# JettHuang/jet-pbrt

Measured on AMD Instinct MI355X. Metric: Msamples/sec (whole node) + per-pixel L2 vs CPU ref, cornell_box 1024spp, higher is better.
Workload: dtype f32

## Files before the change

### jet-pbrt_amd/csrc/jp_kernels.hip

```cpp
#include "jp_common.h"
#include "jp_tex.h"
#include "jp_env.h"
#include "jp_mis.h"
#include "jp_xbsdf.h"

#include <cstdio>
#include <cstring>
#include <string>
#include <vector>
#include <algorithm>
#include <cmath>
#include <mutex>
#include <thread>
#include "jp_devmem.h"
#include "jp_lbvh.h"
#include "jp_ploc.h"

__global__ void __launch_bounds__(JP_BLOCK) k_raygen(SceneView sc, Queues q, RenderConst rc, DevCounters* cnt)
{
	const unsigned int total = (unsigned int)rc.npix * rc.sbatch;
	const unsigned int nchunks = (total + JP_BLOCK - 1) / JP_BLOCK;
	const unsigned int G = gridDim.x, b = blockIdx.x;
	if (b == 0 && threadIdx.x == 0) { cnt->n_queue[0] = total; cnt->n_queue[1] = 0; cnt->n_shadow = 0; }
	unsigned int filled = 0;
// ... 61 lines not shown
		prims = nodes + 5 * sc.n_nodes;
		for (int i = threadIdx.x; i < 4 * sc.n_nodes; i += JP_BLOCK) nodes[5 * (i >> 2) + (i & 3)] = sc.nodes[i];
		for (int i = threadIdx.x; i < 4 * sc.n_prims; i += JP_BLOCK) prims[5 * (i >> 2) + (i & 3)] = sc.prims[i];
		__syncthreads();
	}
	template <bool kAnyHit> __device__ __forceinline__ int trace(const SceneView&, V3 o, V3 d, float tmin, float& tmax) const
	{ return traverse<kAnyHit, 5>(nodes, prims, o, d, tmin, tmax, stack); }
};
template <typename F> struct SceneAccess<2, F>
{
	float4* prims;
	__device__ __forceinline__ SceneAccess(const SceneView& sc, int)
	{
		prims = s_dyn;
		for (int i = threadIdx.x; i < 4 * sc.n_prims; i += JP_BLOCK) prims[5 * (i >> 2) + (i & 3)] = sc.prims[i];
		__syncthreads();
	}
	template <bool kAnyHit> __device__ __forceinline__ int trace(const SceneView& sc, V3 o, V3 d, float tmin, float& tmax) const
	{ return traverse_flat<kAnyHit, 5, F>(sc.flat, sc.n_flat, sc.n_prims, prims, o, d, tmin, tmax); }
	__device__ __forceinline__ int trace_unbounded(const SceneView& sc, V3 o, V3 d, float tmin, float& tmax) const
	{ return traverse_flat<false, 5, F, true>(sc.flat, sc.n_flat, sc.n_prims, prims, o, d, tmin, tmax); }
};

template <> struct SceneAccess<3>
{
	const float4* prims; unsigned int* stack;
	__device__ __forceinline__ SceneAccess(const SceneView& sc, int) : prims(sc.prims), stack((unsigned int*)s_dyn + threadIdx.x) {}
	template <bool kAnyHit> __device__ __forceinline__ int trace(const SceneView& sc, V3 o, V3 d, float tmin, float& tmax) const
	{ return traverse_wide<kAnyHit>(sc.wide, prims, o, d, tmin, tmax, stack); }
};

template <> struct SceneAccess<4>
{
	WalkStack stack;
	__device__ __forceinline__ SceneAccess(const SceneView&, int depth) { stack.lds = (int*)s_dyn + threadIdx.x; stack.spill = nullptr; stack.cap = depth - 1; stack.stride = 0; }
	template <bool kAnyHit> __device__ __forceinline__ int trace(const SceneView& sc, V3 o, V3 d, float tmin, float& tmax) const
	{ return walk_ray<4, kAnyHit>(sc, o, d, tmin, tmax, stack); }
};

template <> struct SceneAccess<6>
{
	WalkStack stack;
	__device__ __forceinline__ SceneAccess(const SceneView&, int depth) { stack.lds = (int*)s_dyn + threadIdx.x; stack.spill = nullptr; stack.cap = depth - 1; stack.stride = 0; }
	template <bool kAnyHit> __device__ __forceinline__ int trace(const SceneView& sc, V3 o, V3 d, float tmin, float& tmax) const
	{ return walk_ray<6, kAnyHit>(sc, o, d, tmin, tmax, stack); }
};

template <> struct SceneAccess<5>
{
	const float4 *nodes, *prims; int* stack;
	__device__ __forceinline__ SceneAccess(const SceneView& sc, int) : nodes(sc.nodes), prims(sc.prims), stack((int*)s_dyn + threadIdx.x) {}
	template <bool kAnyHit> __device__ __forceinline__ int trace(const SceneView&, V3 o, V3 d, float tmin, float& tmax) const
	{ return traverse_ref<kAnyHit>(nodes, prims, o, d, tmin, tmax, stack); }
};

template <int kMode, typename F = FeatAll>
__global__ void __launch_bounds__(JP_BLOCK) k_extend(SceneView sc, Queues q, int cur, int depth, DevCounters* cnt)
{
	SceneAccess<kMode, F> acc(sc, depth);
	const unsigned int b = blockIdx.x, n = q.blk_q[cur][b], rbase = b * q.R;
	if (b == 0 && threadIdx.x == 0) { cnt->closest += cnt->n_queue[cur]; cnt->n_queue[cur ^ 1] = 0; cnt->n_shadow = 0; }
	unsigned int h = 0;
	float4 ro = make_float4(0, 0, 0, 0), rd = make_float4(0, 0, 1, 0);
	if (threadIdx.x < n) { ro = q.ray_o[cur][rbase + threadIdx.x]; rd = q.ray_d[cur][rbase + threadIdx.x]; }
	for (unsigned int j = threadIdx.x; j < n; j += JP_BLOCK)
	{
		const unsigned int i = rbase + j;
		const float4 co = ro, cd = rd;
		if (j + JP_BLOCK < n) { ro = q.ray_o[cur][i + JP_BLOCK]; rd = q.ray_d[cur][i + JP_BLOCK]; }
		float tmax = JP_INF;
		int hit;
		if constexpr (kMode == 2) hit = acc.trace_unbounded(sc, xyz(co), xyz(cd), 0.001f, tmax);
		else hit = acc.template trace<false>(sc, xyz(co), xyz(cd), 0.001f, tmax);
		q.hit[i] = make_float2(tmax, __int_as_float(hit));
		h += hit >= 0 ? 1u : 0u;
	}
	for (int off = 32; off > 0; off >>= 1) h += __shfl_down(h, off);
	if ((threadIdx.x & 63) == 0 && h) atomicAdd(&cnt->closest_hit, (unsigned long long)h);
}

#ifndef JP_SHADE_TILE
#define JP_SHADE_TILE 8192
#endif
template <bool kTab, bool kPrims, bool kStage, bool kSort, bool kTex, bool kPick, bool kEnv, bool kMis, typename F = FeatAll>
__device__ __forceinline__ void shade_body(SceneView sc, Queues q, RenderConst rc, int cur, DevCounters* cnt, const TexView& tv, const PickView& pv, const EnvView& ev, const MisView& mv)
{
	static_assert(kPick || !kMis, "k_shade: the light strategy's pdf needs the light table");
	static_assert(kTab || !kPrims, "k_shade: primitive records in LDS only together with the tables");
	static_assert(kPick || !kEnv, "k_shade: the map light is an entry of the light table");
	constexpr int kWaves = JP_BLOCK / 64, kMaxSeg = (JP_SHADE_TILE / JP_BLOCK) * kWaves;
	static_assert(JP_SHADE_TILE % JP_BLOCK == 0 && JP_SHADE_TILE <= 65536, "k_shade: tile positions are 16-bit");
	__shared__ unsigned short s_idx[kSort ? JP_SHADE_TILE : 1];
	__shared__ unsigned char s_key[kSort ? JP_SHADE_TILE : 1];
	__shared__ unsigned int s_cnt[kSort ? JP_SHADE_CLASSES * kMaxSeg : 1];
	__shared__ unsigned int s_wsum[kWaves];
	__shared__ unsigned int s_ctr[3];
	const unsigned int lane = threadIdx.x & 63u;
	const int n_tab_l = kPick ? 0 : 2 * sc.n_lights;
	const int n_tab = n_tab_l + 4 * sc.n_mats + (sc.n_mats + 3) / 4, n_tab_all = n_tab + (kPrims ? 8 * sc.n_prims : 0);
	float4* s_lights = s_dyn;
	float4* s_mats = s_lights + n_tab_l;
	int* s_mtype = (int*)(s_mats + 4 * sc.n_mats);
	float4* s_prims = s_dyn + n_tab;
	int4* s_meta = (int4*)(s_prims + 4 * sc.n_prims);
	const float4* s_frames = s_prims + 5 * sc.n_prims;
	float4* s_stage = s_dyn + n_tab_all + threadIdx.x;
	const unsigned int b = blockIdx.x, n = q.blk_q[cur][b];
	const int nxt = cur ^ 1;
#ifdef JP_SHADE_TIMING
	unsigned long long t_acc[10] = { 0, 0, 0, 0, 0, 0, 0, 0, 0, 0 }, t_last = __builtin_amdgcn_s_memtime();
#endif
	if (kTab)
	{
		for (int i = threadIdx.x; i < n_tab_all; i += 2 * JP_BLOCK)
		{
			const bool two = i + JP_BLOCK < n_tab_all;
			const float4 a = sc.shade_tab[i], c2 = two ? sc.shade_tab[i + JP_BLOCK] : a;
			s_dyn[i] = a; if (two) s_dyn[i + JP_BLOCK] = c2;
		}
	}
	if (n == 0) { if (threadIdx.x == 0) { q.blk_q[nxt][b] = 0; q.blk_sh[b] = 0; } return; }
	if (threadIdx.x == 0) { s_ctr[0] = 0; s_ctr[1] = 0; s_ctr[2] = 0; }
	__syncthreads();
	const float4* lights = (kTab && !kPick) ? (const float4*)s_lights : sc.lights;
	const float4* mats = kTab ? (const float4*)s_mats : sc.mats;
	const int* mat_type = kTab ? (const int*)s_mtype : sc.mat_type;
	const float4* prims = kPrims ? (const float4*)s_prims : sc.prims;
	const int4* meta_t = kPrims ? (const int4*)s_meta : sc.meta;
	const unsigned int rbase = b * q.R;
	const unsigned int t0 = 0, count = n;
	JP_TS(0);
	if (kSort)
	{
		constexpr unsigned int seg = kMaxSeg, nctr = JP_SHADE_CLASSES * kMaxSeg;
		const unsigned int tid = threadIdx.x;
		const unsigned int plane = tid & 63u, wave = tid >> 6, npass = (count + JP_BLOCK - 1) / JP_BLOCK;
		const unsigned long long ltm = (1ull << plane) - 1ull;
		#pragma unroll 1
		for (unsigned int r0 = 0; r0 < npass; r0 += 8)
		{
			int pi[8];
			#pragma unroll
			for (int u = 0; u < 8; u++)
			{
				const unsigned int j = (r0 + u) * JP_BLOCK + tid;
				pi[u] = j < count ? __float_as_int(q.hit[rbase + t0 + j].y) : -2;
			}
			#pragma unroll
			for (int u = 0; u < 8; u++)
			{
				const unsigned int r = r0 + u;
				if (r >= npass) break;
				unsigned int key = JP_SHADE_CLASSES;
				if (pi[u] != -2)
				{
					int m = -1; if (pi[u] >= 0) m = meta_t[pi[u]].y;
					key = m >= 0 ? 1u + (unsigned int)mat_type[m] : 0u;
				}
				s_key[r * JP_BLOCK + tid] = (unsigned char)key;
				unsigned int mine = 0;
				#pragma unroll
				for (int c = 0; c < JP_SHADE_CLASSES; c++)
				{
					unsigned int nc = 0;
					if ((rc.class_mask >> c) & 1) nc = (unsigned int)__popcll(__ballot(key == (unsigned int)c));
					if (plane == (unsigned int)c) mine = nc;
				}
				if (plane < JP_SHADE_CLASSES) s_cnt[plane * seg + r * kWaves + wave] = mine;
			}
		}
		__syncthreads();
		{
			static_assert(JP_SHADE_CLASSES * kMaxSeg <= 3 * JP_BLOCK, "k_shade: three counters per thread");
			unsigned int v[3], t = 0;
			#pragma unroll
			for (int i = 0; i < 3; i++)
			{
				const unsigned int at = 3 * tid + i;
				v[i] = (at < nctr && (at % seg) / kWaves < npass) ? s_cnt[at] : 0u; t += v[i];
			}
			unsigned int incl = t;
			#pragma unroll
			for (int off = 1; off < 64; off <<= 1) { const unsigned int o = __shfl_up(incl, off); if (plane >= (unsigned int)off) incl += o; }
			if (plane == 63) s_wsum[wave] = incl;
			__syncthreads();
			unsigned int base = incl - t;
			#pragma unroll
			for (int w = 0; w < kWaves; w++) if ((unsigned int)w < wave) base += s_wsum[w];
			#pragma unroll
			for (int i = 0; i < 3; i++) { const unsigned int at = 3 * tid + i; if (at < nctr) s_cnt[at] = base; base += v[i]; }
		}
		__syncthreads();
		#pragma unroll 1
		for (unsigned int r = 0; r < npass; r++)
		{
			const unsigned int key = s_key[r * JP_BLOCK + tid];
			unsigned int pre = 0;
			#pragma unroll
			for (int c = 0; c < JP_SHADE_CLASSES; c++)
			{
				if (!((rc.class_mask >> c) & 1)) continue;
				const unsigned long long m = __ballot(key == (unsigned int)c);
				if (key == (unsigned int)c) pre = (unsigned int)__popcll(m & ltm);
			}
			if (key < JP_SHADE_CLASSES) s_idx[s_cnt[key * seg + r * kWaves + wave] + pre] = (unsigned short)(r * JP_BLOCK + tid);
		}
		__syncthreads();
	}
	float4 ro_n = make_float4(0, 0, 0, 0), rd_n = ro_n, rb_n = ro_n; float2 h_n = make_float2(0, 0); unsigned int s_n = 0; float2 m_n = make_float2(0, 0);
	JP_TS(1);
	const unsigned int nch = (count + 63u) >> 6;
	unsigned int tk = wave_take(&s_ctr[0], 1u);
	unsigned int c0 = (nch - 1u - tk) << 6;
	if (tk < nch && c0 + lane < count) { const unsigned int pos = c0 + lane, i0 = rbase + t0 + (kSort ? (unsigned int)s_idx[pos] : pos); ro_n = q.ray_o[cur][i0]; rd_n = q.ray_d[cur][i0]; rb_n = q.beta[cur][i0]; h_n = q.hit[i0]; if (kTex) s_n = tv.side[i0]; if (kMis) m_n = mv.side[cur][i0]; }
	while (tk < nch)
	{
		const bool valid = c0 + lane < count;
#ifdef JP_SHADE_TIMING
		JP_TS(2);
		asm volatile("s_waitcnt vmcnt(0)" ::: "memory");
		JP_TS(3);
#endif
#ifdef JP_SHADE_NO_PREFETCH
		if (valid) { const unsigned int pos = c0 + lane, i0 = rbase + t0 + (kSort ? (unsigned int)s_idx[pos] : pos); ro_n = q.ray_o[cur][i0]; rd_n = q.ray_d[cur][i0]; rb_n = q.beta[cur][i0]; h_n = q.hit[i0]; if (kTex) s_n = tv.side[i0]; if (kMis) m_n = mv.side[cur][i0]; }
		const float4 ro = ro_n, rd = rd_n, rb = rb_n; const float2 h = h_n; const unsigned int sw = s_n; const float2 ms = m_n;
		tk = wave_take(&s_ctr[0], 1u); c0 = (nch - 1u - tk) << 6;
#else
		const float4 ro = ro_n, rd = rd_n, rb = rb_n; const float2 h = h_n; const unsigned int sw = s_n; const float2 ms = m_n;
		tk = wave_take(&s_ctr[0], 1u); c0 = (nch - 1u - tk) << 6;
		if (tk < nch && c0 + lane < count)
		{
			const unsigned int pos = c0 + lane;
			const unsigned int i1 = rbase + t0 + (kSort ? (unsigned int)s_idx[pos] : pos);
			ro_n = q.ray_o[cur][i1]; rd_n = q.ray_d[cur][i1]; rb_n = q.beta[cur][i1]; h_n = q.hit[i1]; if (kTex) s_n = tv.side[i1]; if (kMis) m_n = mv.side[cur][i1];
		}
#endif
		bool shaded = false, wantNee = false, alive = false;
		V3 o = mk(0, 0, 0), d = mk(0, 0, 1), beta = mk(0, 0, 0), p = mk(0, 0, 0), N = mk(0, 0, 1);
		int slot = 0, bounce = 0; bool spec = false; unsigned int dim = 0; uint32_t key = 0;
		Closure c; c.kind = CL_LAMBERT; Frame fr; fr.s = fr.t = fr.n = mk(0, 0, 1);
		float2 nm = make_float2(0.f, 0.f);
		if (valid)
		{
			o = xyz(ro); d = xyz(rd); beta = xyz(rb);
			slot = __float_as_int(ro.w); key = (uint32_t)__float_as_int(rb.w);
			const int flags = __float_as_int(rd.w);
			bounce = FLAG_BOUNCE(flags); spec = FLAG_SPEC(flags); dim = FLAG_DIM(flags);
			const int pi = __float_as_int(h.y);
			const bool found = pi >= 0;
			int mat = -1, hitprim = 0; bool nflip = false, tabframe = kPrims;
			V3 Le = splat(0);
			float wLe = 1.f;
			if (found)
			{
				const float4 g3 = prims[4 * pi + 3];
				const int4 meta = meta_t[pi];
				const int type = __float_as_int(g3.w);
				p = o + h.x * d;
				if (type == JP_SHAPE_TRIANGLE) N = xyz(g3);
				else if (!F::curved || type == JP_SHAPE_RECTANGLE) { nflip = !(dot(xyz(g3), d) <= 0); N = nflip ? -xyz(g3) : xyz(g3); }
				else if (type == JP_SHAPE_DISK) N = xyz(prims[4 * pi + 1]);
				else { const float4 g0 = prims[4 * pi]; N = normalize(p - xyz(g0)); tabframe = false; }
				hitprim = pi;
				mat = meta.y;
				if (meta.z >= 0 && (bounce == 0 || spec))
				{
					const V3 wo = -d;
					if (dot(N, wo) > 0.f) Le = xyz(lights[2 * meta.z]);
				}
				else if (kMis && meta.z >= 0)
				{
					const V3 wo = -d;
					if (dot(N, wo) > 0.f)
					{
						Le = xyz(lights[2 * meta.z]);
						if (!isblack(Le))
						{
							bool unweighed;
							const float a = light_pdf(sc, prims, lights, pv, ev, kEnv, meta.z, o - ms.y * d, d, ms.y + h.x, N, unweighed);
							wLe = unweighed ? 0.f : (a > 0.f ? mis_weight(ms.x, a) : 1.f);
						}
					}
				}
			}
			else if (F::other_lights && (bounce == 0 || spec))
			{
				if (kEnv)
				{
					const float4 t = ev.texel[env_lookup(ev, d)];
					float4 L = q.lacc[slot];
					V3 a = mk(L.x, L.y, L.z) + cmul(beta, xyz(t));
					q.lacc[slot] = make_float4(a.x, a.y, a.z, 0.f);
				}
				else if (kPick)
				{
					for (int e = 0; e < pv.n_env; e++)
					{
						float4 L = q.lacc[slot];
						V3 a = mk(L.x, L.y, L.z) + cmul(beta, xyz(pv.env[e]));
						q.lacc[slot] = make_float4(a.x, a.y, a.z, 0.f);
					}
				}
				else for (int li = 0; li < sc.n_lights; li++)
				{
					const float4 l0 = lights[2 * li];
					if (__float_as_int(l0.w) == JP_LIGHT_ENVIRONMENT && !isblack(xyz(l0)))
					{
						float4 L = q.lacc[slot];
						V3 a = mk(L.x, L.y, L.z) + cmul(beta, xyz(l0));
						q.lacc[slot] = make_float4(a.x, a.y, a.z, 0.f);
					}
				}
			}
			else if (kMis)
			{
// ... 104 lines not shown
							s_stage[(2 * k) * JP_BLOCK] = make_float4(sdir.x, sdir.y, sdir.z, dist - 0.001f);
							s_stage[(2 * k + 1) * JP_BLOCK] = make_float4(contrib.x, contrib.y, contrib.z, 0.f);
						}
						else
						{
							q.sh_d[(size_t)k * q.cap + qs] = make_float4(sdir.x, sdir.y, sdir.z, dist - 0.001f);
							q.sh_c[(size_t)k * q.cap + qs] = make_float4(contrib.x, contrib.y, contrib.z, 0.f);
						}
						k++;
					}
				}
				if (!kStage) q.sh_o[qs] = make_float4(p.x, p.y, p.z, __int_as_float(slot | (k << rc.slot_bits)));
			}
		}
		JP_TS(5);
#ifdef JP_DBG_SKIP_SAMPLE
		if (false)
#else
		if (shaded)
#endif
		{
			const float ux = rngf(rc, key, dim), uy = rngf(rc, key, dim + 1); dim += 2;
			BsdfSample bs = sample_local<F>(c, wo, ux, uy);
			bs.wi = to_world(fr, bs.wi);
			if (!(isblack(bs.f) || bs.pdf == 0.f))
			{
				nspec = (bs.flags & BS_SPECULAR) != 0;
				if (bounce >= 3)
				{
					const float qq = smax(0.05f, 1 - maxcomp(bs.f));
					const float ur = rngf(rc, key, dim++);
					if (!(ur < qq))
					{
						nbeta = cmul(beta, bs.f * absdot(bs.wi, N) / (bs.pdf * (1 - qq)));
						alive = true;
					}
				}
				else
				{
					nbeta = cmul(beta, bs.f * absdot(bs.wi, N) / bs.pdf);
					alive = true;
				}
				nd = bs.wi; nbounce = bounce + 1;
				if (kMis) nm = make_float2(bs.pdf, 0.f);
			}
		}
		JP_TS(6);
		unsigned int j = 0;
		const unsigned long long lt = (1ull << lane) - 1ull;
		const unsigned long long ma = __ballot(alive);
		if (kStage)
		{
			const unsigned long long ms = __ballot(k > 0);
			if (ma | ms)
			{
				const unsigned int base = wave_take(&s_ctr[1], (unsigned int)__popcll(ma) | ((unsigned int)__popcll(ms) << 16));
				j = rbase + (base & 0xffffu) + (unsigned int)__popcll(ma & lt);
				qs = rbase + (base >> 16) + (unsigned int)__popcll(ms & lt);
			}
			if (k > 0)
			{
				q.sh_o[qs] = make_float4(p.x, p.y, p.z, __int_as_float(slot | (k << rc.slot_bits)));
				for (int kk = 0; kk < k; kk++)
				{
					q.sh_d[(size_t)kk * q.cap + qs] = s_stage[(2 * kk) * JP_BLOCK];
					q.sh_c[(size_t)kk * q.cap + qs] = s_stage[(2 * kk + 1) * JP_BLOCK];
				}
			}
		}
		else if (ma) j = rbase + wave_take(&s_ctr[1], (unsigned int)__popcll(ma)) + (unsigned int)__popcll(ma & lt);
		if (alive)
		{
			q.ray_o[nxt][j] = make_float4(p.x, p.y, p.z, __int_as_float(slot));
			q.ray_d[nxt][j] = make_float4(nd.x, nd.y, nd.z, __int_as_float(MK_FLAGS(nbounce, nspec, dim)));
			q.beta[nxt][j] = make_float4(nbeta.x, nbeta.y, nbeta.z, __int_as_float((int)key));
			if (kMis) mv.side[nxt][j] = nm;
		}
		JP_TS(7);
#ifdef JP_SHADE_TIMING
		asm volatile("s_waitcnt vmcnt(0)" ::: "memory");
		JP_TS(9);
#endif
	}
	JP_TS(2);
	__syncthreads();
	JP_TS(8);
#ifdef JP_SHADE_TIMING
	if (lane == 0) for (int i = 0; i < 10; i++) atomicAdd(&g_shade_t[i], t_acc[i]);
	if (lane == 0) atomicAdd(&g_shade_t[15], 1ull);
#endif
	if (threadIdx.x == 0)
	{
		const unsigned int run_q = kStage ? (s_ctr[1] & 0xffffu) : s_ctr[1], run_sh = kStage ? (s_ctr[1] >> 16) : s_ctr[2];
		q.blk_q[nxt][b] = run_q; q.blk_sh[b] = run_sh;
		if (run_q) atomicAdd(&cnt->n_queue[nxt], run_q);
		if (run_sh) atomicAdd(&cnt->n_shadow, run_sh);
	}
}
template <bool kTab, bool kPrims, bool kStage, bool kSort, typename F = FeatAll>
__global__ void __launch_bounds__(JP_BLOCK) k_shade(SceneView sc, Queues q, RenderConst rc, int cur, DevCounters* cnt)
{
	const TexView tv = {}; const PickView pv = {}; const EnvView ev = {}; const MisView mv = {};
	shade_body<kTab, kPrims, kStage, kSort, false, false, false, false, F>(sc, q, rc, cur, cnt, tv, pv, ev, mv);
}

template <int kMode, typename F = FeatAll>
__global__ void __launch_bounds__(JP_BLOCK, 4) k_shadow(SceneView sc, Queues q, RenderConst rc, int depth, DevCounters* cnt)
{
#ifdef JP_TRAV_TIMING
	unsigned long long t_acc[10] = { 0, 0, 0, 0, 0, 0, 0, 0, 0, 0 }, t_last = __builtin_amdgcn_s_memtime();
#endif
	SceneAccess<kMode, F> acc(sc, depth);
	const unsigned int b = blockIdx.x, E = q.blk_sh[b], rbase = b * q.R;
	JP_TT(0);
	unsigned int rays = 0, occ = 0;
	float4 so_n = make_float4(0, 0, 0, 0), sd_n = make_float4(0, 0, 1, 0);
	if (threadIdx.x < E) { so_n = q.sh_o[rbase + threadIdx.x]; sd_n = q.sh_d[rbase + threadIdx.x]; }
	for (unsigned int j = threadIdx.x; j < E; j += JP_BLOCK)
	{
		const unsigned int e = rbase + j;
#ifdef JP_TRAV_TIMING
		JP_TT(1);
		asm volatile("s_waitcnt vmcnt(0)" ::: "memory");
		JP_TT(2);
#endif
		const float4 so = so_n; float4 sd = sd_n;
		if (j + JP_BLOCK < E) { so_n = q.sh_o[e + JP_BLOCK]; sd_n = q.sh_d[e + JP_BLOCK]; }
		const int packed = __float_as_int(so.w);
		const int slot = packed & ((1 << rc.slot_bits) - 1), n = (int)((unsigned int)packed >> rc.slot_bits);
		if (n == 0) continue;
		bool any = false;
		const float4 L = q.lacc[slot];
		V3 a = mk(L.x, L.y, L.z);
		for (int k = 0; k < n; k++)
		{
			const float4 c4 = q.sh_c[(size_t)k * q.cap + e];
			float tmax = sd.w;
			const V3 dir = xyz(sd);
			if (k + 1 < n) sd = q.sh_d[(size_t)(k + 1) * q.cap + e];
			JP_TT(3);
#ifdef JP_TRAV_TIMING
			int hit;
			if constexpr (kMode == 2)
			{
				unsigned int m;
				if constexpr (F::curved) m = flat_boxes<false>(sc.flat, sc.n_flat, xyz(so), dir, 0.001f, tmax);
				else m = flat_boxes_lean<false>(sc.flat, sc.n_flat, xyz(so), dir, 0.001f, tmax);
				JP_TT(4);
				hit = flat_prims<true, false, 5, F>(m, acc.prims, xyz(so), dir, 0.001f, tmax);
				JP_TT(5);
			}
			else hit = acc.template trace<true>(sc, xyz(so), dir, 0.001f, tmax);
#else
			const int hit = acc.template trace<true>(sc, xyz(so), dir, 0.001f, tmax);
#endif
			rays++;
			if (hit >= 0) occ++;
			else { a = a + xyz(c4); any = true; }
			JP_TT(6);
		}
		if (any) q.lacc[slot] = make_float4(a.x, a.y, a.z, 0.f);
		JP_TT(7);
	}
#ifdef JP_TRAV_TIMING
	JP_TT(1);
	if ((threadIdx.x & 63) == 0) { for (int i = 0; i < 8; i++) atomicAdd(&g_shade_t[i], t_acc[i]); atomicAdd(&g_shade_t[15], 1ull); }
#endif
	for (int off = 32; off > 0; off >>= 1) { rays += __shfl_down(rays, off); occ += __shfl_down(occ, off); }
	if ((threadIdx.x & 63) == 0) { if (rays) atomicAdd(&cnt->shadow, (unsigned long long)rays); if (occ) atomicAdd(&cnt->shadow_occ, (unsigned long long)occ); }
}

template <int kMode, bool kAnyHit, bool kVote>
__device__ __forceinline__ void persist_turn(Walker<kMode>& w, const SceneView& sc, const WalkStack& stack, bool pool)
{
	const int nh = __popcll(__ballot(!w.done && w.heavy())), nl = __popcll(__ballot(!w.done && !w.heavy()));
	const bool heavyTurn = kVote ? nh > nl : w.heavy();
	if (kVote) { JP_TURN(heavyTurn ? 3 : 0, 1); JP_TURN(heavyTurn ? 4 : 1, heavyTurn ? nh : nl); JP_TURN(heavyTurn ? 5 : 2, nh + nl); if (!pool) { JP_TURN(8, 1); JP_TURN(9, nh + nl); JP_TURN(10, heavyTurn ? nh : nl); } }
	if (!w.done && (w.heavy() == heavyTurn)) w.template step<kAnyHit>(sc, stack);
}
__device__ __forceinline__ unsigned int lane_rank(unsigned long long m) { return __builtin_amdgcn_mbcnt_hi((unsigned int)(m >> 32), __builtin_amdgcn_mbcnt_lo((unsigned int)m, 0u)); }

#ifndef JP_CERT_WAVES
#define JP_CERT_WAVES 8
#endif
template <int kMode, int kRefill, bool kVote>
__global__ void __launch_bounds__(JP_BLOCK, (kMode == 6 ? JP_CERT_WAVES : 8)) k_extend_persist(SceneView sc, Queues q, int cur_q, int stack_cap, int* spill, DevCounters* cnt)
// ... 477 lines not shown
```

### jet-pbrt_amd/csrc/jp_render.h

```cpp
#pragma once
namespace
{
enum { CLS_EXTEND = 0, CLS_SHADE = 1, CLS_SHADOW = 2, CLS_OTHER = 3, CLS_PATH = 4 };

void free_queues(JpContext* c) { c->qb = QueueBufs(); c->cap = 0; c->planes_alloc = 0; c->blk_alloc = 0; }

int ensure_queues(JpContext* c, unsigned int cap, int planes, unsigned int nblocks)
{
	if (c->cap >= cap && c->planes_alloc >= planes && c->blk_alloc >= nblocks) return JP_OK;
	cap = std::max(cap, c->cap); planes = std::max(planes, c->planes_alloc); nblocks = std::max(nblocks, c->blk_alloc);
	free_queues(c);
	auto alloc = [](DevBuf& b, auto*& p, size_t bytes) { return reserve(b, p, bytes) == hipSuccess; };
	Queues& q = c->q; QueueBufs& qb = c->qb; bool ok = true;
	for (int b = 0; b < 2 && ok; b++) ok = alloc(qb.ray_o[b], q.ray_o[b], (size_t)cap * 16) && alloc(qb.ray_d[b], q.ray_d[b], (size_t)cap * 16) && alloc(qb.beta[b], q.beta[b], (size_t)cap * 16)
	                                       && alloc(qb.blk_q[b], q.blk_q[b], (size_t)nblocks * 4);
	ok = ok && alloc(qb.hit, q.hit, (size_t)cap * 8) && alloc(qb.lacc, q.lacc, (size_t)cap * 16) && alloc(qb.sh_o, q.sh_o, (size_t)cap * 16)
	     && alloc(qb.sh_d, q.sh_d, (size_t)cap * 16 * planes) && alloc(qb.sh_c, q.sh_c, (size_t)cap * 16 * planes) && alloc(qb.blk_sh, q.blk_sh, (size_t)nblocks * 4);
	if (!ok) { free_queues(c); return fail(JP_ERR_DEVICE, "jp_render: out of device memory for the path queues"); }
	c->cap = cap; c->planes_alloc = planes; c->blk_alloc = nblocks;
	return JP_OK;
}

int ensure_gamma(JpContext* c)
{
// ... 28 lines not shown
{
	if (rp->width <= 0 || rp->height <= 0 || rp->spp <= 0 || rp->max_depth < 0 || rp->max_depth > 200) return fail(JP_ERR_INVALID_ARGUMENT, "jp_render: bad width/height/spp/max_depth");
	if (rp->integrator < JP_INTEGRATOR_PATH || rp->integrator > JP_INTEGRATOR_DEBUG_NORMAL) return fail(JP_ERR_INVALID_ARGUMENT, "jp_render: unknown integrator");
	if (rp->integrator == JP_INTEGRATOR_WHITTED && rp->max_depth > JP_WHITTED_MAX_DEPTH) return fail(JP_ERR_UNSUPPORTED, "jp_render: the Whitted integrator supports max_depth <= 16");
	if (rp->sampler_mode != JP_SAMPLER_COUNTER && rp->sampler_mode != JP_SAMPLER_DEBUG) return fail(JP_ERR_UNSUPPORTED, "jp_render: the device path implements the counter sampler only (the sequential mt19937_64 stream is not reproducible in parallel)");
	s.band = rp->band_rows > 0 ? rp->band_rows : 20;
	s.count = rp->shard_count > 1 ? rp->shard_count : 1;
	s.index = s.count > 1 ? rp->shard_index : 0;
	if (s.index < 0 || s.index >= s.count) return fail(JP_ERR_INVALID_ARGUMENT, "jp_render: shard_index out of range");
	const int nbands = (rp->height + s.band - 1) / s.band;
	s.local_rows = 0;
	for (int b = s.index; b < nbands; b += s.count) s.local_rows += std::min(s.band, rp->height - b * s.band);
	s.lane_rows = 0;
	for (int g0 = lane_index * lane_group; g0 < s.local_rows; g0 += lane_count * lane_group) s.lane_rows += std::min(lane_group, s.local_rows - g0);
	return JP_OK;
}

inline bool refill_walks(const ScenePlan& p) { return p.persist && (p.trav_mode == 0 || p.trav_mode == 3 || p.trav_mode == 5); }
inline int refill_row(const ScenePlan& p) { return p.persist >= 32 ? 2 : (p.persist >= 16 ? 1 : 0); }
inline int extend_depth(const ScenePlan& p) { return (p.trav_mode == 5 ? p.cert : p.use_q4) ? p.stack_depth_q4 : p.stack_depth; }
inline int shadow_depth(const ScenePlan& p) { return (p.trav_mode == 5 ? p.cert : p.q4_shadow) ? p.stack_depth_q4 : (p.trav_mode == 3 ? (int)(p.lds_bytes_shadow / (JP_BLOCK * sizeof(int))) : p.stack_depth); }
inline int deepest_walk(const ScenePlan& p) { return std::max(std::max(p.stack_depth, p.stack_depth_q4), p.trav_mode == 3 ? (int)(p.lds_bytes_shadow / (JP_BLOCK * sizeof(int))) : 0); }
inline size_t spill_need(const ScenePlan& p, int deep, unsigned int G) { return deep >= p.stack_lds_words ? (size_t)(deep - p.stack_lds_words + 1) * G * JP_BLOCK : 1; }

inline bool flat_shapes_only(int shape_mask) { return (shape_mask & ~((1 << JP_SHAPE_TRIANGLE) | (1 << JP_SHAPE_RECTANGLE))) == 0; }
inline bool lean_traversal(const ScenePlan& p, bool generic) { return !generic && p.trav_mode == 2 && flat_shapes_only(p.shape_mask); }
inline bool lean_shading(const ScenePlan& p, bool generic)
{
	const int delta_classes = (2 << JP_MAT_MIRROR) | (2 << JP_MAT_GLASS) | (2 << JP_MAT_PLASTIC);
	return !generic && p.shade_prims_in_lds && p.stage_nee && flat_shapes_only(p.shape_mask) && (p.light_mask & ~(1 << JP_LIGHT_AREA)) == 0
	    && flat_shapes_only(p.light_shape_mask) && (p.class_mask & delta_classes) == 0;
}

typedef void (*ExtendKernel)(SceneView, Queues, int, int, DevCounters*);
typedef void (*ExtendRefillKernel)(SceneView, Queues, int, int, int*, DevCounters*);
struct ExtendLaunch { ExtendRefillKernel refill; ExtendKernel plain; size_t lds; int words; };
template <int M> ExtendRefillKernel extend_refill(const ScenePlan& p)
{
	static const ExtendRefillKernel k[3][2] = { { k_extend_persist<M, 8, false>, k_extend_persist<M, 8, true> }, { k_extend_persist<M, 16, false>, k_extend_persist<M, 16, true> }, { k_extend_persist<M, 32, false>, k_extend_persist<M, 32, true> } };
	return k[refill_row(p)][p.vote];
}
ExtendLaunch extend_kernel(const ScenePlan& p, bool generic)
{
	if (lean_traversal(p, generic)) return { nullptr, k_extend<2, FeatFlat>, p.lds_bytes, p.stack_depth };
	if (!refill_walks(p)) return { nullptr, p.trav_mode == 5 ? k_extend<5> : (p.trav_mode == 2 ? k_extend<2> : (p.trav_mode == 1 ? k_extend<1> : k_extend<0>)), p.lds_bytes, p.stack_depth };
	const int words = std::min(extend_depth(p), p.stack_lds_words);
	const ExtendRefillKernel k = p.trav_mode == 5 ? (p.cert ? extend_refill<6>(p) : extend_refill<5>(p)) : (p.use_q4 ? extend_refill<4>(p) : extend_refill<0>(p));
	return { k, nullptr, (size_t)words * JP_BLOCK * sizeof(int), words };
}

typedef void (*ShadowKernel)(SceneView, Queues, RenderConst, int, DevCounters*);
typedef void (*ShadowRefillKernel)(SceneView, Queues, RenderConst, int, int*, DevCounters*);
struct ShadowLaunch { ShadowRefillKernel refill; ShadowKernel plain; size_t lds; int words; bool cert_fell_back; };
template <int M> ShadowRefillKernel shadow_refill(const ScenePlan& p)
{
	static const ShadowRefillKernel k[3][2] = { { k_shadow_persist<M, 8, false>, k_shadow_persist<M, 8, true> }, { k_shadow_persist<M, 16, false>, k_shadow_persist<M, 16, true> }, { k_shadow_persist<M, 32, false>, k_shadow_persist<M, 32, true> } };
	return k[refill_row(p)][p.vote];
}
ShadowLaunch shadow_kernel(const ScenePlan& p, unsigned int R, bool generic)
{
	const int words = std::min(shadow_depth(p), p.stack_lds_words);
	const size_t plds = (size_t)words * JP_BLOCK * sizeof(int) + (((size_t)R * p.n_planes + 31) / 32) * 4 * (p.cert ? 2 : 1);
	if (lean_traversal(p, generic)) return { nullptr, k_shadow<2, FeatFlat>, p.lds_bytes, p.stack_depth, p.cert };
	if (!refill_walks(p) || plds > 64 * 1024)
		return { nullptr, p.trav_mode == 3 ? k_shadow<3> : (p.trav_mode == 5 ? k_shadow<5> : (p.trav_mode == 2 ? k_shadow<2> : (p.trav_mode == 1 ? k_shadow<1> : k_shadow<0>))), p.trav_mode == 3 ? p.lds_bytes_shadow : p.lds_bytes, p.stack_depth, p.cert };
	const ShadowRefillKernel k = p.trav_mode == 5 ? (p.cert ? shadow_refill<6>(p) : shadow_refill<5>(p)) : (p.q4_shadow ? shadow_refill<4>(p) : (p.trav_mode == 3 ? shadow_refill<3>(p) : shadow_refill<0>(p)));
	return { k, nullptr, plds, words, false };
}

typedef void (*ShadeKernel)(SceneView, Queues, RenderConst, int, DevCounters*);
typedef void (*ShadeTexKernel)(SceneView, Queues, RenderConst, int, DevCounters*, TexView);
struct ShadeKernels { ShadeKernel plain; ShadeTexKernel tex; };
template <bool kTab, bool kPrims, bool kStage> ShadeKernels shade_row(bool sort)
{
	ShadeKernels k = { sort ? k_shade<kTab, kPrims, kStage, true> : k_shade<kTab, kPrims, kStage, false>, sort ? k_shade_tex<kTab, kPrims, kStage, true> : k_shade_tex<kTab, kPrims, kStage, false> };
	return k;
}
ShadeKernels shade_kernels(const ScenePlan& p, bool generic)
{
	if (lean_shading(p, generic))
	{
		ShadeKernels k = shade_row<true, true, true>(p.shade_sort);
		k.plain = p.shade_sort ? k_shade<true, true, true, true, FeatLean> : k_shade<true, true, true, false, FeatLean>;
		return k;
	}
	if (p.shade_prims_in_lds) return p.stage_nee ? shade_row<true, true, true>(p.shade_sort) : shade_row<true, true, false>(p.shade_sort);
	if (p.tables_in_lds) return p.stage_nee ? shade_row<true, false, true>(p.shade_sort) : shade_row<true, false, false>(p.shade_sort);
	return shade_row<false, false, false>(p.shade_sort);
}

typedef void (*ShadePickKernel)(SceneView, Queues, RenderConst, int, DevCounters*, PickView);
typedef void (*ShadePickTexKernel)(SceneView, Queues, RenderConst, int, DevCounters*, TexView, PickView);
struct ShadePickKernels { ShadePickKernel plain; ShadePickTexKernel tex; };
ShadePickKernels shade_pick_kernels(const ScenePlan& p);
typedef void (*ShadeEnvKernel)(SceneView, Queues, RenderConst, int, DevCounters*, PickView, EnvView);
typedef void (*ShadeEnvTexKernel)(SceneView, Queues, RenderConst, int, DevCounters*, TexView, PickView, EnvView);
struct ShadeEnvKernels { ShadeEnvKernel plain; ShadeEnvTexKernel tex; };
ShadeEnvKernels shade_env_kernels(const ScenePlan& p);
typedef void (*ShadeMisKernel)(SceneView, Queues, RenderConst, int, DevCounters*, PickView, MisView);
typedef void (*ShadeMisTexKernel)(SceneView, Queues, RenderConst, int, DevCounters*, TexView, PickView, MisView);
typedef void (*ShadeMisEnvKernel)(SceneView, Queues, RenderConst, int, DevCounters*, PickView, EnvView, MisView);
typedef void (*ShadeMisEnvTexKernel)(SceneView, Queues, RenderConst, int, DevCounters*, TexView, PickView, EnvView, MisView);
struct ShadeMisKernels { ShadeMisKernel pick; ShadeMisTexKernel pick_tex; ShadeMisEnvKernel env; ShadeMisEnvTexKernel env_tex; };
ShadeMisKernels shade_mis_kernels(const ScenePlan& p);
}
static int ensure_mis_side(JpContext* c, unsigned int cap, MisView& mv);
namespace
{

typedef void (*OtherKernel)(SceneView, Queues, RenderConst, int, int, DevCounters*);
OtherKernel other_kernel(const ScenePlan& p) { return p.trav_mode == 5 ? k_other<5> : (p.trav_mode == 2 ? k_other<2> : (p.trav_mode == 1 ? k_other<1> : k_other<0>)); }

typedef void (*TraceKernel)(SceneView, int, int, const float*, const float*, const float*, const float*, int*, float*, int*, float*);
typedef void (*SurfaceKernel)(SceneView, TexView, int, int, const float*, const float*, const float*, const float*, int*, float*, float*);
struct TraceLaunch { TraceKernel trace; SurfaceKernel surface; size_t lds; int depth; };
template <int M> TraceLaunch trace_row(size_t lds, int depth) { TraceLaunch t = { k_trace<M>, k_surface<M>, lds, depth }; return t; }
TraceLaunch trace_kernel(const ScenePlan& p, int tw, bool generic = true)
{
	const size_t q4lds = (size_t)p.stack_depth_q4 * JP_BLOCK * sizeof(int);
	if (p.trav_mode == 3 && tw == 2) { TraceLaunch t = { k_trace<3>, nullptr, p.lds_bytes_shadow, p.stack_depth }; return t; }
	if (p.trav_mode == 5 && p.cert && q4lds <= 64 * 1024 && tw != 3) return trace_row<6>(q4lds, p.stack_depth_q4);
	if (p.trav_mode == 5) return trace_row<5>(p.lds_bytes, p.stack_depth);
	if (p.use_q4 && q4lds <= 64 * 1024 && tw != 1) return trace_row<4>(q4lds, p.stack_depth_q4);
	if (lean_traversal(p, generic)) { TraceLaunch t = { k_trace_flat, k_surface<2>, p.lds_bytes, p.stack_depth }; return t; }
	return p.trav_mode == 2 ? trace_row<2>(p.lds_bytes, p.stack_depth) : (p.trav_mode == 1 ? trace_row<1>(p.lds_bytes, p.stack_depth) : trace_row<0>(p.lds_bytes, p.stack_depth));
}

int render_one(JpContext* c, const JpRenderParams* rp, float* film_dev, bool sync, int lane_index = 0, int lane_count = 1, int lane_group = 4, bool ev0_recorded = false)
{
	if (!c->plan.have_scene) return fail(JP_ERR_NO_SCENE, "jp_render: no scene uploaded");
	const ScenePlan& p = c->plan; Shard sh; DevCounters* const d_cnt = c->cnt.get<DevCounters>();
	if (const int e = shard_of(rp, sh, lane_index, lane_count, lane_group); e != JP_OK) return e;
	HIP_TRY(hipSetDevice(c->device));
	const long long npix = (long long)sh.lane_rows * rp->width;

	if (!ev0_recorded) HIP_TRY(hipEventRecord(c->ev0, c->stream));
	HIP_TRY(hipMemsetAsync(film_dev, 0, sizeof(float) * 3 * (size_t)rp->width * rp->height, c->stream));
	HIP_TRY(hipMemsetAsync(d_cnt, 0, sizeof(DevCounters), c->stream));
	c->evused = 0; c->stamps.clear();
	unsigned long long samples = 0;
	if (npix > 0)
	{
		if (npix > (1 << 24)) return fail(JP_ERR_UNSUPPORTED, "jp_render: more than 2^24 pixels per shard");
		const int slot_bits = p.n_planes <= 31 ? 27 : 24;
		const unsigned int PMAX = slot_bits == 27 ? (1u << 26) : (1u << 24);
		size_t freeB = 0, totalB = 0; hipMemGetInfo(&freeB, &totalB);
		const size_t per = 136 + 32 * (size_t)p.n_planes;
		size_t budget = std::min<size_t>((size_t)24 << 30, (freeB / (size_t)std::max(1, lane_count) + (c->cap ? (size_t)c->cap * (136 + 32 * (size_t)c->planes_alloc) : 0)) / 2);
		if (c->opt.max_slots > 0) budget = std::min<size_t>(budget, (size_t)c->opt.max_slots * per);
		int sbatch = 1; unsigned int P = 0, G = 1, R = JP_BLOCK, cap = 0;
		for (int attempt = 0;; attempt++)
		{
			const unsigned int pcap = (unsigned int)std::min<size_t>(PMAX, std::max<size_t>((size_t)npix, budget / per));
			sbatch = (int)std::max<long long>(1, std::min<long long>(rp->spp, pcap / npix));
			{
				const int nb = (rp->spp + sbatch - 1) / sbatch;
				sbatch = (rp->spp + nb - 1) / nb;
			}
			if ((long long)sbatch * npix > (long long)PMAX) return fail(JP_ERR_UNSUPPORTED, "jp_render: shard too large for one batch");
			P = (unsigned int)((long long)sbatch * npix);
			const unsigned int nchunks = (P + JP_BLOCK - 1) / JP_BLOCK;
			G = std::max(1u, std::min(nchunks, (unsigned int)(c->n_cus * c->blocks_per_cu)));
			G = std::max(G, (nchunks + JP_SHADE_TILE / JP_BLOCK - 1) / (JP_SHADE_TILE / JP_BLOCK));
			R = ((nchunks + G - 1) / G) * JP_BLOCK;
			cap = G * R;
			const int st = ensure_queues(c, cap, p.n_planes, G);
// ... 529 lines not shown
```

### jet-pbrt_amd/csrc/jp_shading.h

```cpp
#pragma once
#include "jp_device.h"
#define JP_HD_INLINE __host__ __device__ __forceinline__

namespace jp
{
__device__ __forceinline__ void sincos_d(float xf, double* s, double* c)
{
	const double x = (double)xf;
	const double kd = rint(x * 0.63661977236758134308);
	const int k = (int)kd;
	double r = fma(-kd, 1.57079632679489655800e+00, x);
	r = fma(-kd, 6.12323399573676603587e-17, r);
	const double r2 = r * r;
	double sp = fma(r2, -7.6471637318198164759e-13, 1.6059043836821614599e-10);
	sp = fma(sp, r2, -2.5052108385441718775e-08);
	sp = fma(sp, r2, 2.7557319223985890653e-06);
	sp = fma(sp, r2, -1.9841269841269841270e-04);
	sp = fma(sp, r2, 8.3333333333333333333e-03);
	sp = fma(sp, r2, -1.6666666666666666667e-01);
	sp = fma(sp * r2, r, r);
	double cp = fma(r2, 4.7794773323873852974e-14, -1.1470745597729724714e-11);
	cp = fma(cp, r2, 2.0876756987868098979e-09);
	cp = fma(cp, r2, -2.7557319223985890653e-07);
	cp = fma(cp, r2, 2.4801587301587301587e-05);
// ... 303 lines not shown
				float cos_t = sqrtf(1 - sin2_t);
				s.wi = eta * -wo + (eta * cos_i - cos_t) * n;
				V3 ft = c.c1 * (1 - F);
				ft = ft * ((etaI * etaI) / (etaT * etaT));
				s.pdf = 1 - F;
				s.f = ft / fabsf(s.wi.z);
				s.flags = BS_TRANSMISSION | BS_SPECULAR;
			}
		}
	}
	else
	{
		if (wo.z == 0) return s;
		V3 wh = tr_sample_wh(c, wo, ux, uy);
		float owh = dot(wo, wh);
		if (owh < 0) return s;
		V3 wi = -wo + 2 * owh * wh;
		if (!same_hemi(wo, wi)) return s;
		s.wi = wi;
		s.f = eval_local<FS>(c, wo, wi);
		s.pdf = tr_Pdf(c, wo, wh) / (4 * dot(wo, wh));
		s.flags = BS_REFLECTION | BS_GLOSSY;
	}
	return s;
}

template <typename F = FeatAll, typename MatPtr>
__device__ __forceinline__ void make_closure(MatPtr mats, int type, int mat, float uplastic, Closure& c)
{
	const float4 p0 = mats[4 * mat + 0], p1 = mats[4 * mat + 1];
	c.c0 = splat(0); c.c1 = splat(0); c.eta_t = 1; c.ax = c.ay = 0; c.fresnel = FR_CONDUCTOR; c.feta = splat(0); c.fk = splat(0);
	if (type == JP_MAT_MATTE) { c.kind = CL_LAMBERT; c.c0 = xyz(p0); }
	else if (F::delta && type == JP_MAT_MIRROR) { c.kind = CL_MIRROR; c.c0 = xyz(p0); }
	else if (F::delta && type == JP_MAT_GLASS) { c.kind = CL_FRESNEL_SPECULAR; c.eta_t = p0.x; c.c0 = mk(p0.y, p0.z, p0.w); c.c1 = mk(p1.x, p1.y, p1.z); }
	else if (F::delta && type == JP_MAT_PLASTIC)
	{
		float Qd = p1.w;
		if (uplastic < Qd) { c.kind = CL_LAMBERT; c.c0 = xyz(p0) / Qd; }
		else { c.kind = CL_MICROFACET; c.c0 = mk(p0.w, p1.x, p1.y) / (1 - Qd); c.fresnel = FR_DIELECTRIC; c.ax = c.ay = smax(0.001f, p1.z); }
	}
	else { c.kind = CL_MICROFACET; c.c0 = splat(1.f); c.fresnel = FR_CONDUCTOR; c.feta = xyz(p0); c.fk = mk(p0.w, p1.x, p1.y); c.ax = smax(0.001f, p1.z); c.ay = smax(0.001f, p1.w); }
}

struct LightSample { V3 pos, wi; float pdf; V3 Li; float dist; };

template <typename F = FeatAll, typename PrimPtr, typename LightPtr>
__device__ __forceinline__ LightSample sample_li(const SceneView& sc, PrimPtr prims, LightPtr lights, int li, V3 p, V3 n_isect, float ux, float uy)
{
	LightSample s; s.pos = mk(0, 0, 0); s.wi = mk(0, 0, 0); s.pdf = 0; s.Li = splat(0); s.dist = -1.f;
	const float4 l0 = lights[2 * li], l1 = lights[2 * li + 1];
	const V3 radiance = xyz(l0);
	if (F::other_lights && __float_as_int(l0.w) == JP_LIGHT_ENVIRONMENT)
	{
		float theta = uy * JP_PI, phi = ux * 2 * JP_PI;
		float cosT, sinT, sinP, cosP; sincos_f(theta, &sinT, &cosT); sincos_f(phi, &sinP, &cosP);
		s.wi = mk(sinT * cosP, sinT * sinP, cosT);
		s.pos = p + s.wi * 2 * sc.world_radius;
		if (sinT != 0) s.pdf = 1 / (2 * JP_PI * JP_PI * sinT);
		s.Li = radiance;
		return s;
	}
	if (F::other_lights && __float_as_int(l0.w) == JP_LIGHT_POINT)
	{
		const V3 wp = xyz(l1);
		s.pos = wp;
		s.wi = normalize(wp - p);
		s.pdf = 1.f;
		s.Li = radiance / len2(wp - p);
		return s;
	}
	if (F::other_lights && __float_as_int(l0.w) == JP_LIGHT_DIRECTION)
	{
		s.wi = -xyz(l1);
		s.pos = p + s.wi * 2 * sc.world_radius;
		s.pdf = 1.f;
		s.Li = radiance;
		return s;
	}
	const int pi = __float_as_int(l1.x);
	const float inv_area = l1.y;
	const float4 g0 = prims[4 * pi + 0], g3 = prims[4 * pi + 3];
	const int type = __float_as_int(g3.w);
	V3 lp, ln; float pdf;
	if (!F::other_lights || type != JP_SHAPE_SPHERE)
	{
		const float4 g1 = prims[4 * pi + 1], g2 = prims[4 * pi + 2];
		if (type == JP_SHAPE_TRIANGLE)
		{
			float su0 = sqrtf(ux); float bx = 1 - su0, by = uy * su0;
			lp = bx * xyz(g0) + by * xyz(g1) + (1 - bx - by) * xyz(g2);
		}
		else if (F::other_lights && type == JP_SHAPE_DISK)
		{
			const Frame fr = frame_from_z(xyz(g1));
			float px, py; concentric_disk(ux, uy, px, py);
			lp = xyz(g0) + g0.w * (fr.s * px + fr.t * py);
		}
		else lp = xyz(g1) + (xyz(g0) - xyz(g1)) * ux + (xyz(g2) - xyz(g1)) * uy;
		ln = (F::other_lights && type == JP_SHAPE_DISK) ? xyz(g1) : xyz(g3);
		pdf = inv_area;
		V3 wi = lp - p;
		float dist2 = len2(wi);
		if (dist2 == 0) pdf = 0;
		else
		{
			const float l = sqrtf(dist2);
			wi = wi / l;
			s.dist = l;
			pdf *= dist2 / absdot(ln, -wi);
			if (isinf(pdf)) pdf = 0;
		}
	}
	else
	{
		const V3 c = xyz(g0); const float r = g0.w;
		if (len2(p - c) <= r * r)
		{
			V3 dir = uniform_sphere(ux, uy);
			lp = c + r * dir; ln = normalize(dir);
			pdf = inv_area;
			V3 wi = lp - p;
			if (len2(wi) == 0) pdf = 0;
			else { wi = normalize(wi); pdf *= len2(lp - p) / absdot(n_isect, -wi); }
			if (isinf(pdf)) pdf = 0;
		}
		else
		{
			float dist = len(p - c);
			float inv_dist = 1 / dist;
			float sin_max = r * inv_dist;
			float sin_max2 = sin_max * sin_max;
			float inv_sin_max = 1 / sin_max;
			float cos_max = sqrtf(smax(0.f, 1 - sin_max2));
			float cos_theta = (cos_max - 1) * ux + 1;
			float sin_theta2 = 1 - cos_theta * cos_theta;
			if (sin_max2 < 0.00068523f) { sin_theta2 = sin_max2 * ux; cos_theta = sqrtf(1 - sin_theta2); }
			float cos_alpha = sin_theta2 * inv_sin_max + cos_theta * sqrtf(smax(0.f, 1.f - sin_theta2 * inv_sin_max * inv_sin_max));
			float sin_alpha = sqrtf(smax(0.f, 1.f - cos_alpha * cos_alpha));
			float phi = uy * 2 * JP_PI;
			Frame fr = frame_from_z((c - p) * inv_dist);
			float sphi, cphi; sincos_f(phi, &sphi, &cphi);
			V3 wn = sin_alpha * cphi * (-fr.s) + sin_alpha * sphi * (-fr.t) + cos_alpha * (-fr.n);
			lp = c + r * wn; ln = wn;
			pdf = 1 / (2 * JP_PI * (1 - cos_max));
		}
	}
	s.pos = lp; s.pdf = pdf;
	if (pdf == 0 || len2(lp - p) == 0) s.Li = splat(0);
	else
	{
		s.wi = normalize(lp - p);
		s.Li = (dot(ln, -s.wi) > 0.f) ? radiance : splat(0);
	}
	return s;
}

}
```

Before: 3117.

## Partition shade queue in one sweep into matte and metal ends; reuse light direction

Result: faster. 3281 (median of 6 runs) (+5.3%).

```diff
diff --git a/jet-pbrt_amd/csrc/jp_kernels.hip b/jet-pbrt_amd/csrc/jp_kernels.hip
--- a/jet-pbrt_amd/csrc/jp_kernels.hip
+++ b/jet-pbrt_amd/csrc/jp_kernels.hip
@@ -167,7 +167,7 @@
 #ifndef JP_SHADE_TILE
 #define JP_SHADE_TILE 8192
 #endif
-template <bool kTab, bool kPrims, bool kStage, bool kSort, bool kTex, bool kPick, bool kEnv, bool kMis, typename F = FeatAll>
+template <bool kTab, bool kPrims, bool kStage, bool kSort, bool kTex, bool kPick, bool kEnv, bool kMis, typename F = FeatAll, bool kOne = false>
 __device__ __forceinline__ void shade_body(SceneView sc, Queues q, RenderConst rc, int cur, DevCounters* cnt, const TexView& tv, const PickView& pv, const EnvView& ev, const MisView& mv)
 {
 	static_assert(kPick || !kMis, "k_shade: the light strategy's pdf needs the light table");
@@ -176,8 +176,10 @@
 	constexpr int kWaves = JP_BLOCK / 64, kMaxSeg = (JP_SHADE_TILE / JP_BLOCK) * kWaves;
 	static_assert(JP_SHADE_TILE % JP_BLOCK == 0 && JP_SHADE_TILE <= 65536, "k_shade: tile positions are 16-bit");
 	__shared__ unsigned short s_idx[kSort ? JP_SHADE_TILE : 1];
-	__shared__ unsigned char s_key[kSort ? JP_SHADE_TILE : 1];
-	__shared__ unsigned int s_cnt[kSort ? JP_SHADE_CLASSES * kMaxSeg : 1];
+	static_assert(!kOne || (kSort && kPrims && !F::delta && !F::other_lights && !kTex && !kPick && !kMis), "k_shade: the one-sweep partition is the lean sorted instance's");
+	__shared__ unsigned char s_key[kSort && !kOne ? JP_SHADE_TILE : 1];
+	__shared__ unsigned int s_cnt[kSort && !kOne ? JP_SHADE_CLASSES * kMaxSeg : 1];
+	__shared__ unsigned int s_two;
 	__shared__ unsigned int s_wsum[kWaves];
 	__shared__ unsigned int s_ctr[3];
 	const unsigned int lane = threadIdx.x & 63u;
@@ -205,7 +207,7 @@
 		}
 	}
 	if (n == 0) { if (threadIdx.x == 0) { q.blk_q[nxt][b] = 0; q.blk_sh[b] = 0; } return; }
-	if (threadIdx.x == 0) { s_ctr[0] = 0; s_ctr[1] = 0; s_ctr[2] = 0; }
+	if (threadIdx.x == 0) { s_ctr[0] = 0; s_ctr[1] = 0; s_ctr[2] = 0; if (kOne) s_two = 0; }
 	__syncthreads();
 	const float4* lights = (kTab && !kPick) ? (const float4*)s_lights : sc.lights;
 	const float4* mats = kTab ? (const float4*)s_mats : sc.mats;
@@ -215,7 +217,47 @@
 	const unsigned int rbase = b * q.R;
 	const unsigned int t0 = 0, count = n;
 	JP_TS(0);
-	if (kSort)
+	if (kOne)
+	{
+		const unsigned int tid = threadIdx.x, npass = (count + JP_BLOCK - 1) / JP_BLOCK;
+		const unsigned long long ltm = (1ull << lane) - 1ull;
+		#pragma unroll 1
+		for (unsigned int r0 = 0; r0 < npass; r0 += 8)
+		{
+			int pi[8];
+			#pragma unroll
+			for (int u = 0; u < 8; u++)
+			{
+				const unsigned int j = (r0 + u) * JP_BLOCK + tid;
+				pi[u] = j < count ? __float_as_int(q.hit[rbase + t0 + j].y) : -2;
+			}
+			int mt[8]; unsigned long long ma[8], mb[8];
+			unsigned int na = 0, nb = 0;
+			#pragma unroll
+			for (int u = 0; u < 8; u++)
+			{
+				mt[u] = -1;
+				if (pi[u] >= 0) { const int m = meta_t[pi[u]].y; if (m >= 0) mt[u] = mat_type[m]; }
+				ma[u] = __ballot(mt[u] == JP_MAT_MATTE); mb[u] = __ballot(mt[u] == JP_MAT_METAL);
+				na += (unsigned int)__popcll(ma[u]); nb += (unsigned int)__popcll(mb[u]);
+			}
+			if (na | nb)
+			{
+				const unsigned int base = wave_take(&s_two, na | (nb << 16));
+				unsigned int a = base & 0xffffu, m = base >> 16;
+				#pragma unroll
+				for (int u = 0; u < 8; u++)
+				{
+					const unsigned short j = (unsigned short)((r0 + u) * JP_BLOCK + tid);
+					if (mt[u] == JP_MAT_MATTE) s_idx[a + (unsigned int)__popcll(ma[u] & ltm)] = j;
+					if (mt[u] == JP_MAT_METAL) s_idx[count - 1u - (m + (unsigned int)__popcll(mb[u] & ltm))] = j;
+					a += (unsigned int)__popcll(ma[u]); m += (unsigned int)__popcll(mb[u]);
+				}
+			}
+		}
+		__syncthreads();
+	}
+	else if (kSort)
 	{
 		constexpr unsigned int seg = kMaxSeg, nctr = JP_SHADE_CLASSES * kMaxSeg;
 		const unsigned int tid = threadIdx.x;
@@ -294,28 +336,31 @@
 	}
 	float4 ro_n = make_float4(0, 0, 0, 0), rd_n = ro_n, rb_n = ro_n; float2 h_n = make_float2(0, 0); unsigned int s_n = 0; float2 m_n = make_float2(0, 0);
 	JP_TS(1);
-	const unsigned int nch = (count + 63u) >> 6;
+	const unsigned int n_front = kOne ? (s_two & 0xffffu) : 0u, n_back = kOne ? (s_two >> 16) : 0u, fence = ((n_front + 63u) >> 6) << 6;
+#define JP_CHUNK_HAS(v)  (kOne ? ((v) < fence ? (v) < n_front : (v) - fence < n_back) : (v) < count)
+#define JP_CHUNK_SPOT(v) (kOne ? ((v) < fence ? (v) : count - 1u - ((v) - fence)) : (v))
+	const unsigned int nch = kOne ? (fence >> 6) + ((n_back + 63u) >> 6) : (count + 63u) >> 6;
 	unsigned int tk = wave_take(&s_ctr[0], 1u);
 	unsigned int c0 = (nch - 1u - tk) << 6;
-	if (tk < nch && c0 + lane < count) { const unsigned int pos = c0 + lane, i0 = rbase + t0 + (kSort ? (unsigned int)s_idx[pos] : pos); ro_n = q.ray_o[cur][i0]; rd_n = q.ray_d[cur][i0]; rb_n = q.beta[cur][i0]; h_n = q.hit[i0]; if (kTex) s_n = tv.side[i0]; if (kMis) m_n = mv.side[cur][i0]; }
+	if (tk < nch && JP_CHUNK_HAS(c0 + lane)) { const unsigned int pos = JP_CHUNK_SPOT(c0 + lane), i0 = rbase + t0 + (kSort ? (unsigned int)s_idx[pos] : pos); ro_n = q.ray_o[cur][i0]; rd_n = q.ray_d[cur][i0]; rb_n = q.beta[cur][i0]; h_n = q.hit[i0]; if (kTex) s_n = tv.side[i0]; if (kMis) m_n = mv.side[cur][i0]; }
 	while (tk < nch)
 	{
-		const bool valid = c0 + lane < count;
+		const bool valid = JP_CHUNK_HAS(c0 + lane);
 #ifdef JP_SHADE_TIMING
 		JP_TS(2);
 		asm volatile("s_waitcnt vmcnt(0)" ::: "memory");
 		JP_TS(3);
 #endif
 #ifdef JP_SHADE_NO_PREFETCH
-		if (valid) { const unsigned int pos = c0 + lane, i0 = rbase + t0 + (kSort ? (unsigned int)s_idx[pos] : pos); ro_n = q.ray_o[cur][i0]; rd_n = q.ray_d[cur][i0]; rb_n = q.beta[cur][i0]; h_n = q.hit[i0]; if (kTex) s_n = tv.side[i0]; if (kMis) m_n = mv.side[cur][i0]; }
+		if (valid) { const unsigned int pos = JP_CHUNK_SPOT(c0 + lane), i0 = rbase + t0 + (kSort ? (unsigned int)s_idx[pos] : pos); ro_n = q.ray_o[cur][i0]; rd_n = q.ray_d[cur][i0]; rb_n = q.beta[cur][i0]; h_n = q.hit[i0]; if (kTex) s_n = tv.side[i0]; if (kMis) m_n = mv.side[cur][i0]; }
 		const float4 ro = ro_n, rd = rd_n, rb = rb_n; const float2 h = h_n; const unsigned int sw = s_n; const float2 ms = m_n;
 		tk = wave_take(&s_ctr[0], 1u); c0 = (nch - 1u - tk) << 6;
 #else
 		const float4 ro = ro_n, rd = rd_n, rb = rb_n; const float2 h = h_n; const unsigned int sw = s_n; const float2 ms = m_n;
 		tk = wave_take(&s_ctr[0], 1u); c0 = (nch - 1u - tk) << 6;
-		if (tk < nch && c0 + lane < count)
-		{
-			const unsigned int pos = c0 + lane;
+		if (tk < nch && JP_CHUNK_HAS(c0 + lane))
+		{
+			const unsigned int pos = JP_CHUNK_SPOT(c0 + lane);
 			const unsigned int i1 = rbase + t0 + (kSort ? (unsigned int)s_idx[pos] : pos);
 			ro_n = q.ray_o[cur][i1]; rd_n = q.ray_d[cur][i1]; rb_n = q.beta[cur][i1]; h_n = q.hit[i1]; if (kTex) s_n = tv.side[i1]; if (kMis) m_n = mv.side[cur][i1];
 		}
@@ -586,6 +631,8 @@
 		JP_TS(9);
 #endif
 	}
+#undef JP_CHUNK_HAS
+#undef JP_CHUNK_SPOT
 	JP_TS(2);
 	__syncthreads();
 	JP_TS(8);
@@ -606,6 +653,11 @@
 {
 	const TexView tv = {}; const PickView pv = {}; const EnvView ev = {}; const MisView mv = {};
 	shade_body<kTab, kPrims, kStage, kSort, false, false, false, false, F>(sc, q, rc, cur, cnt, tv, pv, ev, mv);
+}
+__global__ void __launch_bounds__(JP_BLOCK) k_shade_lean_one(SceneView sc, Queues q, RenderConst rc, int cur, DevCounters* cnt)
+{
+	const TexView tv = {}; const PickView pv = {}; const EnvView ev = {}; const MisView mv = {};
+	shade_body<true, true, true, true, false, false, false, false, FeatLean, true>(sc, q, rc, cur, cnt, tv, pv, ev, mv);
 }
 
 template <int kMode, typename F = FeatAll>
diff --git a/jet-pbrt_amd/csrc/jp_render.h b/jet-pbrt_amd/csrc/jp_render.h
--- a/jet-pbrt_amd/csrc/jp_render.h
+++ b/jet-pbrt_amd/csrc/jp_render.h
@@ -134,6 +134,9 @@
 	{
 		ShadeKernels k = shade_row<true, true, true>(p.shade_sort);
 		k.plain = p.shade_sort ? k_shade<true, true, true, true, FeatLean> : k_shade<true, true, true, false, FeatLean>;
+#ifndef JP_NO_ONE_SWEEP
+		if (p.shade_sort && !p.has_null_material) k.plain = k_shade_lean_one;
+#endif
 		return k;
 	}
 	if (p.shade_prims_in_lds) return p.stage_nee ? shade_row<true, true, true>(p.shade_sort) : shade_row<true, true, false>(p.shade_sort);
diff --git a/jet-pbrt_amd/csrc/jp_shading.h b/jet-pbrt_amd/csrc/jp_shading.h
--- a/jet-pbrt_amd/csrc/jp_shading.h
+++ b/jet-pbrt_amd/csrc/jp_shading.h
@@ -409,6 +409,9 @@
 	const float4 g0 = prims[4 * pi + 0], g3 = prims[4 * pi + 3];
 	const int type = __float_as_int(g3.w);
 	V3 lp, ln; float pdf;
+#ifndef JP_NO_KEEP_WI
+	V3 kept = mk(0, 0, 0); bool have_kept = false;
+#endif
 	if (!F::other_lights || type != JP_SHAPE_SPHERE)
 	{
 		const float4 g1 = prims[4 * pi + 1], g2 = prims[4 * pi + 2];
@@ -434,6 +437,9 @@
 			const float l = sqrtf(dist2);
 			wi = wi / l;
 			s.dist = l;
+#ifndef JP_NO_KEEP_WI
+			kept = wi; have_kept = true;
+#endif
 			pdf *= dist2 / absdot(ln, -wi);
 			if (isinf(pdf)) pdf = 0;
 		}
@@ -476,6 +482,10 @@
 	if (pdf == 0 || len2(lp - p) == 0) s.Li = splat(0);
 	else
 	{
+#ifndef JP_NO_KEEP_WI
+		if (!F::other_lights || have_kept) s.wi = kept;
+		else
+#endif
 		s.wi = normalize(lp - p);
 		s.Li = (dot(ln, -s.wi) > 0.f) ? radiance : splat(0);
 	}
```
